# neggles/neurosis

Hardware: AMD Instinct MI355X
Metric: train images/sec (node) SDXL 1024^2 (higher is better)
Workload: dtype bf16

## Files before the change

include/neurosis_hip.h:

```cpp
#ifndef NEUROSIS_HIP_H
#define NEUROSIS_HIP_H

#ifdef __cplusplus
extern "C" {
#endif

const char* nk_last_error(void);
int nk_abi_version(void);

int nk_linear_fwd(const void* x, const void* w, const float* bias, const void* residual, void* y,
                  int M, int N, int K, long ldx, long ldw, long ldr, long ldy, float alpha, void* stream);
int nk_linear_dgrad(const void* dy, const void* w, const void* dx_add, void* dx, int M, int N, int K,
                    long lddy, long ldw, long ldadd, long lddx, void* stream);
long nk_linear_fwd_geglu_ok(int M, int I, int K);
int nk_linear_fwd_geglu(const void* x, const void* w, const float* bias, void* u, void* h, int M, int I, int K, long ldx, long ldw, long ldu,
                        long ldh, void* stream);
int nk_linear_dgrad_geglu(const void* dy, const void* w, const void* u, void* du, int M, int N, int I, long lddy, long ldw, long ldu,
                          long lddu, void* stream);
int nk_linear_fwd_geglu_s(const void* x, const void* w, const float* bias, void* s, void* h, int M, int I, int K, long ldx, long ldw, long lds,
                          long ldh, void* stream);
int nk_linear_dgrad_geglu_s(const void* dy, const void* w, const void* s, void* du, int M, int N, int I, long lddy, long ldw, long lds,
                            long lddu, void* stream);
int nk_linear_wgrad(const void* dy, const void* x, float* dw, int M, int N, int K, long lddy, long ldx,
                    long lddw, int accumulate, void* stream);
// ... 84 lines not shown
long nk_layernorm_ws_floats(int M, int C);
int nk_rmsnorm_fwd(const void* x, const float* gamma, void* y, int M, int C, float eps, void* stream);
int nk_layernorm_bwd(const void* dy, const void* x, const float* gamma, const float* mean, const float* rstd,
                     const void* dx_add, void* dx, float* dgamma, float* dbeta, float* ws, int M, int C, int accumulate, void* stream);
#define NK_COLPART_MAX 32
typedef struct NkColpartBatch {
  const float* part[NK_COLPART_MAX];
  float* dgamma[NK_COLPART_MAX];
  float* dbeta[NK_COLPART_MAX];
  int nrows[NK_COLPART_MAX];
  int C[NK_COLPART_MAX];
  int accumulate[NK_COLPART_MAX];
  int n;
} NkColpartBatch;
long nk_layernorm_part_rows(int M);
int nk_layernorm_bwd_rows(const void* dy, const void* x, const float* gamma, const float* mean, const float* rstd,
                          const void* dx_add, void* dx, float* part, int M, int C, void* stream);
int nk_colpart_reduce_batch(const NkColpartBatch* b, void* stream);
int nk_layernorm_bwd_dx(const void* dy, const void* x, const float* gamma, const float* mean, const float* rstd,
                        const void* dx_add, void* dx, int M, int C, void* stream);
int nk_layernorm_bwd_params(const void* dy, const void* x, const float* mean, const float* rstd, float* dgamma,
                            float* dbeta, float* ws, int M, int C, int accumulate, void* stream);

int nk_geglu_fwd(const void* u, void* y, long M, int I, void* stream);
int nk_geglu_bwd(const void* dy, const void* u, void* du, long M, int I, void* stream);
int nk_geglu_fwd_s(const void* u, void* y, void* s, long M, int I, void* stream);
int nk_geglu_bwd_s(const void* dy, const void* s, void* du, long M, int I, void* stream);

int nk_silu_fwd(const void* x, void* y, long n, void* stream);
int nk_silu_bwd(const void* dy, const void* x, void* dx, long n, void* stream);

int nk_dropout(const void* x, const void* residual, void* y, long rows, int cols, long ld_x, long ld_res, long ld_y, const void* token,
               int site, int thr, float scale, void* stream);
int nk_dropout_draw(void* state, void* token, void* stream);

int nk_add(const void* a, const void* b, void* out, long n, void* stream);

int nk_cat_channels(const void* a, const void* b, void* out, long rows, int Ca, int Cb, void* stream);
int nk_split_channels(const void* src, void* a, void* b, long rows, int Ca, int Cb, void* stream);

int nk_upsample2x_bwd(const void* dup, void* dx, int N, int H, int W, int C, void* stream);
int nk_upsample2x_fwd(const void* x, void* up, int N, int H, int W, int C, void* stream);
int nk_avgpool2x_fwd(const void* x, void* y, int N, int H, int W, int C, void* stream);
int nk_avgpool2x_bwd(const void* dy, void* dx, int N, int H, int W, int C, void* stream);

int nk_nchw_to_nhwc(const void* src, int src_is_f32, void* dst, int N, int C, int HW, int Cpad, float scale,
// ... 119 lines not shown
```

neurosis_amd/lib.py:

```python
from __future__ import annotations

import ctypes as C
import os
from pathlib import Path

import torch

CSRC = Path(__file__).resolve().parent / "csrc"
LIB_PATH = CSRC / "libneurosis_hip.so"

vp, i32, i64, f32 = C.c_void_p, C.c_int, C.c_long, C.c_float


class NkConvDesc(C.Structure):
    _fields_ = [(n, i32) for n in ("N", "H", "W", "Cin", "Cout", "KH", "KW", "stride", "pad_t", "pad_l", "Ho", "Wo", "upsample")]


class NkAttnDesc(C.Structure):
    _fields_ = (
        [(n, i32) for n in ("B", "H", "Lq", "Lk", "D")]
        + [(n, i64) for n in ("sq", "sk", "sv", "so", "bq", "bk", "bv", "bo", "sdq", "sdk", "sdv", "sdo", "bdq", "bdk", "bdv", "bdo")]
        + [("scale", f32), ("causal", i32)]
    )


NK_COLPART_MAX = 32


class NkColpartBatch(C.Structure):
    _fields_ = [("part", vp * NK_COLPART_MAX), ("dgamma", vp * NK_COLPART_MAX), ("dbeta", vp * NK_COLPART_MAX), ("nrows", i32 * NK_COLPART_MAX),
                ("C", i32 * NK_COLPART_MAX), ("accumulate", i32 * NK_COLPART_MAX), ("n", i32)]


cdp, adp = C.POINTER(NkConvDesc), C.POINTER(NkAttnDesc)

SIGNATURES: dict[str, list] = {
    "nk_linear_fwd": [vp, vp, vp, vp, vp, i32, i32, i32, i64, i64, i64, i64, f32, vp],
    "nk_linear_dgrad": [vp, vp, vp, vp, i32, i32, i32, i64, i64, i64, i64, vp],
    "nk_linear_dgrad_geglu": [vp, vp, vp, vp, i32, i32, i32, i64, i64, i64, i64, vp],
    "nk_linear_fwd_geglu": [vp, vp, vp, vp, vp, i32, i32, i32, i64, i64, i64, i64, vp],
    "nk_linear_fwd_geglu_s": [vp, vp, vp, vp, vp, i32, i32, i32, i64, i64, i64, i64, vp],
    "nk_linear_dgrad_geglu_s": [vp, vp, vp, vp, i32, i32, i32, i64, i64, i64, i64, vp],
    "nk_linear_wgrad": [vp, vp, vp, i32, i32, i32, i64, i64, i64, i32, vp],
    "nk_linear_fwd_batched": [C.POINTER(vp), C.POINTER(vp), C.POINTER(vp), i32, i32, i32, i32, i64, i64, i64, vp],
    "nk_linear_wgrad_batched": [C.POINTER(vp), C.POINTER(vp), C.POINTER(vp), C.POINTER(vp), i32, i32, i32, i32, i64, i64, i64, i32, vp],
    "nk_linear_wgrad_bias": [vp, vp, vp, vp, i32, i32, i32, i64, i64, i64, i32, vp],
    "nk_conv2d_wgrad_bias": [cdp, vp, vp, vp, vp, i32, vp],
    "nk_conv2d_fwd": [cdp, vp, vp, vp, vp, vp, vp, vp],
    "nk_conv2d_fwd_stats": [cdp, vp, vp, vp, vp, vp, vp, vp, i32, vp],
    "nk_conv_weight_flip": [vp, vp, i32, i32, i32, vp],
    "nk_conv3x3_few_channels_fwd": [vp, vp, vp, vp, i32, i32, i32, i32, i32, vp],
    "nk_conv2d_dgrad": [cdp, vp, vp, vp, vp],
    "nk_conv2d_dgrad_flipped": [cdp, vp, vp, vp, vp],
    "nk_conv2d_wgrad": [cdp, vp, vp, vp, i32, vp],
# ... 2 lines not shown
    "nk_attention_bwd_causal": [adp, vp, vp, vp, vp, vp, vp, vp, vp, vp, vp],
    "nk_attention_relbias_fwd": [adp, vp, vp, vp, vp, vp, vp],
    "nk_softmax_rows": [vp, i64, i32, vp],
    "nk_softmax_rows_bwd": [vp, vp, i64, i32, f32, vp],
    "nk_groupnorm_fwd": [vp, vp, vp, vp, vp, vp, vp, i32, i32, i32, i32, f32, i32, vp],
    "nk_groupnorm_sums": [vp, vp, vp, i32, i32, i32, i32, vp],
    "nk_groupnorm_sums_from_parts": [vp, vp, vp, i32, i32, i32, vp],
    "nk_groupnorm_apply": [vp, vp, vp, vp, vp, vp, vp, i32, i32, i32, i32, f32, i32, vp],
    "nk_groupnorm_bwd": [vp, vp, vp, vp, vp, vp, vp, vp, vp, vp, vp, i32, i32, i32, i32, i32, i32, vp],
    "nk_groupnorm_mod_fwd": [vp, vp, vp, vp, vp, vp, vp, vp, i32, i32, i32, i32, f32, i32, vp],
    "nk_groupnorm_mod_apply": [vp, vp, vp, vp, vp, vp, vp, vp, i32, i32, i32, i32, f32, i32, vp],
    "nk_groupnorm_mod_bwd": [vp, vp, vp, vp, vp, vp, vp, vp, vp, vp, vp, vp, vp, i32, i32, i32, i32, i32, i32, vp],
    "nk_layernorm_fwd": [vp, vp, vp, vp, vp, vp, i32, i32, f32, vp],
    "nk_rmsnorm_fwd": [vp, vp, vp, i32, i32, f32, vp],
    "nk_layernorm_bwd": [vp, vp, vp, vp, vp, vp, vp, vp, vp, vp, i32, i32, i32, vp],
    "nk_layernorm_bwd_dx": [vp, vp, vp, vp, vp, vp, vp, i32, i32, vp],
    "nk_layernorm_bwd_rows": [vp, vp, vp, vp, vp, vp, vp, vp, i32, i32, vp],
    "nk_colpart_reduce_batch": [C.POINTER(NkColpartBatch), vp],
    "nk_layernorm_bwd_params": [vp, vp, vp, vp, vp, vp, vp, i32, i32, i32, vp],
    "nk_geglu_fwd": [vp, vp, i64, i32, vp],
    "nk_geglu_bwd": [vp, vp, vp, i64, i32, vp],
    "nk_geglu_fwd_s": [vp, vp, vp, i64, i32, vp],
    "nk_geglu_bwd_s": [vp, vp, vp, i64, i32, vp],
    "nk_silu_fwd": [vp, vp, i64, vp],
    "nk_gelu_fwd": [vp, vp, i64, i32, vp],
    "nk_gated_gelu_tanh_fwd": [vp, vp, i64, i32, vp],
    "nk_gelu_bwd": [vp, vp, vp, i64, i32, vp],
    "nk_embedding_bwd": [vp, vp, i64, vp, vp, i32, i32, i32, i32, i32, i32, vp],
    "nk_gather_rows_bwd": [vp, i64, vp, vp, i32, i32, i32, vp],
    "nk_wgrad_few_rows": [vp, i64, vp, i64, vp, i64, i32, i32, i32, i32, vp],
    "nk_vq_search": [vp, i64, vp, vp, vp, i64, i32, i32, vp],
    "nk_vq_code_stats": [vp, vp, i64, vp, vp, i64, i32, i32, vp],
    "nk_vq_quantize": [vp, vp, vp, i64, vp, vp, vp, i64, i32, i32, i32, vp],
    "nk_leaky_relu_fwd": [vp, vp, i64, f32, vp],
    "nk_leaky_relu_bwd": [vp, vp, vp, i64, f32, vp],
    "nk_maxpool2x2_fwd": [vp, vp, i32, i32, i32, i32, vp],
    "nk_maxpool2x2_bwd": [vp, vp, vp, i32, i32, i32, i32, vp],
    "nk_maxpool_fwd": [vp, vp, i32, i32, i32, i32, i32, i32, vp],
    "nk_maxpool_bwd": [vp, vp, vp, i32, i32, i32, i32, i32, i32, vp],
    "nk_lpips_layer_fwd": [vp, vp, vp, vp, vp, i32, i32, i32, f32, i32, vp],
    "nk_lpips_layer_bwd": [vp, vp, vp, vp, vp, i32, i32, i32, f32, vp],
    "nk_batchnorm_fwd": [vp, vp, vp, vp, vp, vp, vp, vp, vp, i64, i32, f32, f32, f32, vp],
    "nk_batchnorm_bwd": [vp, vp, vp, vp, vp, vp, vp, vp, vp, vp, i64, i32, f32, i32, vp],
    "nk_batchnorm_eval": [vp, vp, vp, vp, vp, vp, vp, i64, i32, f32, f32, vp],
    "nk_silu_bwd": [vp, vp, vp, i64, vp],
    "nk_add": [vp, vp, vp, i64, vp],
# ... 20 lines not shown
    "nk_sample_denoise": [vp, vp, vp, vp, f32, vp, i32, i32, i32, i32, i32, vp],
    "nk_sample_euler_step": [vp, vp, vp, vp, vp, vp, f32, vp, vp, i32, i32, i32, i32, i32, vp],
    "nk_adamw_flat": [vp, vp, vp, vp, vp, i64, f32, f32, f32, f32, f32, i32, f32, vp],
    "nk_ema_flat": [vp, vp, i64, f32, vp],
    "nk_debug_raise_health": [vp],
    "nk_debug_stamp": [vp, vp],
    "nk_debug_launch_log": [i32],
    "nk_health_clear": [],
    "nk_health_export": [vp, vp],
    "nk_health_import": [vp, vp],
    "nk_adafactor_init": [vp, vp],
    "nk_adafactor_chunk": [vp, vp],
    "nk_came_chunk": [vp, vp],
    "nk_adamw8bit_step": [vp, vp],
}

SIZE_QUERIES: dict[str, list] = {
    "nk_groupnorm_ws_floats": [i32, i32, i32, i32],
    "nk_groupnorm_sums_ws_floats": [i32, i32, i32],
    "nk_conv2d_stats_tiles": [cdp, i32],
    "nk_conv2d_dgrad_flipped_ok": [cdp],
    "nk_linear_fwd_geglu_ok": [i32, i32, i32],
    "nk_layernorm_ws_floats": [i32, i32],
    "nk_layernorm_part_rows": [i32],
    "nk_colsum_ws_floats": [i64, i32],
    "nk_batchnorm_ws_floats": [i64, i32],
    "nk_lpips_layer_ws_floats": [i32, i32],
    "nk_attention_bwd_ws_floats": [adp],
    "nk_vq_search_ws_floats": [i64, i32],
    "nk_vq_quantize_ws_floats": [i64],
    "nk_adafactor_tensor_bytes": [],
    "nk_came_tensor_bytes": [],
    "nk_adamw8bit_tensor_bytes": [],
    "nk_gemm_sk_status": [],
    "nk_health_status": [],
    "nk_debug_launch_names": [C.c_char_p, i64],
}

_lib = None


class NkError(RuntimeError):
    pass


def load() -> C.CDLL:
# ... 48 lines not shown
```

neurosis_amd/models/diffusion.py:

```python
from __future__ import annotations

import os
from contextlib import contextmanager, nullcontext
from math import ceil
from typing import Callable, Optional

import torch
from torch import Tensor, nn

from .. import ops
from ..modules.diffusion import Denoiser, DiffusionLoss, OpenAIWrapper, UNetModel
from ..nn import FlatParamStore
from .autoencoder import AutoencoderKL


class PrecomputedConditioner(nn.Module):

    def forward(self, batch: dict, force_zero_embeddings=None) -> dict:
        zeroed = set(force_zero_embeddings or ())
        out = {}
        for k in ("crossattn", "vector", "concat"):
            if k in batch and batch[k] is not None:
                out[k] = torch.zeros_like(batch[k]) if k in zeroed else batch[k]
        return out
# ... 106 lines not shown
        if self.optimizer is not None and self._torch_optimizer is None:
            self.configure_optimizers()
        self.stream_optimizer = self.stream_optimizer
        return self.store

    @property
    def stream_optimizer(self) -> bool:
        return self._stream_optimizer

    @stream_optimizer.setter
    def stream_optimizer(self, on: bool) -> None:
        if on and self.trainable_embedders():
            raise NotImplementedError("stream_optimizer (the update streamed block by block behind backward) does not drive the text towers' groups")
        if on and getattr(self, "_torch_optimizer", None) is not None:
            from ..optimizers import CAME, AdamW8bit

            if isinstance(self._torch_optimizer, (CAME, AdamW8bit)):
                raise NotImplementedError(f"DiffusionEngine: stream_optimizer (the update streamed block by block behind backward) needs the fused "
                                          f"Adafactor, not {type(self._torch_optimizer).__name__}")
        self._stream_optimizer = bool(on)
        unet = getattr(getattr(self, "model", None), "diffusion_model", None)
        if unet is None or getattr(self, "store", None) is None:
            return
        if on:
            if unet.grad_ready_hook is None:
                unet.grad_ready_hook = self._grads_ready
        elif unet.grad_ready_hook == self._grads_ready:
            unet.grad_ready_hook = None

    def _block_boundaries(self) -> list:
        unet = self.model.diffusion_model
        index = {id(p): i for i, p in enumerate(self.store.params)}
        tops = [unet.time_embed, getattr(unet, "label_emb", None), *unet.input_blocks, unet.middle_block, *unet.output_blocks, unet.out]
        out = []
        for m in tops:
            if m is None:
                continue
            idx = [index[id(p)] for p in m.parameters() if id(p) in index]
            if idx:
                out.append(min(idx))
        return sorted(set(out))

    def _grads_ready(self, module: nn.Module) -> None:
        af = getattr(self, "adafactor", None)
        if af is None or not self.stream_optimizer or not self._last_micro_batch or not self.store.master.is_cuda:
            return
# ... 271 lines not shown
```

neurosis_amd/modules/diffusion/openaimodel.py:

```python
from __future__ import annotations

import os

from typing import Callable, List, Optional, Union

import torch
from torch import Tensor, nn

from ... import ops
from ...nn import Conv2d, FlatParamStore, apply_module, as_tokens, linear_module_fwd
from ...ops import BF16, Img
from ..attention import SpatialTransformer, zero_module


def conv_nd(dims: int, *args, **kwargs) -> nn.Module:
    if dims != 2:
        raise ValueError(f"unsupported dimensions: {dims} (the MI355X path implements 2-D convolutions)")
    return Conv2d(*args, **kwargs)


class TimestepBlock(nn.Module):

    def forward(self, x: Tensor, emb: Tensor):
        raise NotImplementedError("TimestepBlock is an interface: subclasses implement forward(x, emb)")
# ... 7 lines not shown
        for layer in self:
            if isinstance(layer, TimestepBlock):
                x, b = layer.fwd(x, emb)
                bwds.append(("emb", b))
            elif isinstance(layer, SpatialTransformer):
                x, b = layer.fwd(x, context, need_dctx=dctx_sink is not None)
                bwds.append(("ctx", b))
            elif isinstance(layer, (Conv2d, Upsample, Downsample)):
                x, b = layer.fwd(x, need_dx=not (first and getattr(self, "_nk_input_block", False)))
                bwds.append(("plain", b))
            elif isinstance(layer, nn.Identity):
                continue
            else:
                raise NotImplementedError(f"TimestepEmbedSequential: unsupported layer {type(layer).__name__}")
            first = False

        def bwd(dy: Tensor):
            demb = None
            for kind, b in reversed(bwds):
                if dy is None:
                    break
                if kind == "emb":
                    dy, de = b(dy)
                    demb = de if demb is None else ops.add(demb, de)
                elif kind == "ctx":
                    dy, dc = b(dy)
                    if dctx_sink is not None and dc is not None:
                        dctx_sink(dc)
                else:
                    dyi, _ = b(dy)
                    dy = None if dyi is None else dyi.t
            bwds.clear()
            return dy, demb

        return x, bwd

    def forward(self, x: Tensor, emb: Tensor, context: Optional[Tensor] = None, image_only_indicator=None, time_context=None, num_video_frames=None):
        ins = [x, emb] if context is None else [x, emb, context]
        ops.dropout_open(self)

        def run(x, emb, context=None):
            img = Img.from_nchw(x)
            out, bwd = self.fwd(img, as_tokens(emb), None if context is None else as_tokens(context))

            def bwd2(g):
                dx, demb = bwd(Img.from_nchw(g).t)
                res = (Img(dx, img.N, img.H, img.W).to_nchw(), None if demb is None else demb.view(emb.shape))
# ... 117 lines not shown
        if isinstance(skip, nn.Identity):
            s, b_skip = x.t, None
        elif skip.kernel_size == 1:
            s, b_skip = ops.linear_fwd(x.t, skip.weight, skip.bias)
        else:
            si, b_skip3 = skip.fwd(x, upsample=self._up)
            s, b_skip = si.t, (lambda g: b_skip3(g)[0].t)
        b_up = None
        if self._up and (b_skip is None or skip.kernel_size == 1):
            sup, b_up = ops.upsample2x_fwd(Img(s, x.N, x.H, x.W))
            s = sup.t
        if b_skip is None and b_res is None and b_up is None:
            return s, None

        def bwd(dy: Tensor) -> Tensor:
            if b_up is not None:
                dy = b_up(dy)
            if b_skip is not None:
                dy = b_skip(dy)
            return dy if b_res is None else b_res(dy)

        return s, bwd

    def _fwd(self, x: Img, emb: Tensor):
        gn1, gn2 = self.in_layers[0], self.out_layers[0]
        ssn = self.use_scale_shift_norm
        h1, b_gn1 = ops.groupnorm_fwd(x, gn1.weight, gn1.bias, 32, gn1.eps, silu=True)
        b_pool = None
        if self._down:
            h1, b_pool = ops.avgpool2x_fwd(h1)
        es, b_es = ops.silu_fwd(emb)
        eo, b_eo = linear_module_fwd(self.emb_layers[1], es)
        h2, b_c1 = self.in_layers[2].fwd(h1, rowvec=None if ssn else eo, upsample=self._up, stats_groups=32)
        if ssn:
            h3, b_gn2 = ops.groupnorm_mod_fwd(h2, gn2.weight, gn2.bias, eo, 32, gn2.eps, silu=True)
        else:
            h3, b_gn2 = ops.groupnorm_fwd(h2, gn2.weight, gn2.bias, 32, gn2.eps, silu=True)
        b_drop = None
        if self.training and self.dropout_p > 0.0:
            _, b_drop = ops.dropout_fwd(h3.t, self.dropout_p, ops.dropout_site(self), inplace=True)
        s, b_skip = self._skip_fwd(x)
        out, b_c2 = self.out_layers[3].fwd(h3, residual=s, stats_groups=32)

        def bwd(dy: Tensor):
            dh3, _ = b_c2(dy)
            dh2 = b_gn2(dh3.t if b_drop is None else b_drop(dh3.t, inplace=True))
            if ssn:
                dh2, deo = dh2
                dh1, _ = b_c1(dh2)
            else:
                dh1, deo = b_c1(dh2)
            dh1 = dh1.t if b_pool is None else b_pool(dh1.t)
            dxs = dy if b_skip is None else b_skip(dy)
            dx = b_gn1(dh1, dxs)
            demb = b_es(b_eo(deo))
            return dx, demb

        return out, bwd

    def fwd(self, x: Img, emb: Tensor):
        if not (self.use_checkpoint and ops.recording()):
            return self._fwd(x, emb)
        out, _ = self._fwd(x, emb)
        tok = ops.dropout_token(required=False)

        def bwd(dy: Tensor):
            with ops.dropout_token_scope(tok):
                _, b = self._fwd(x, emb)
            return b(dy)

        return out, bwd

    def forward(self, x: Tensor, emb: Tensor) -> Tensor:
        ops.dropout_open(self)

        def run(x, emb):
            img = Img.from_nchw(x)
            out, bwd = self.fwd(img, as_tokens(emb))

            def bwd2(g):
                dx, demb = bwd(Img.from_nchw(g).t)
                return Img(dx, img.N, img.H, img.W).to_nchw(), demb.view(emb.shape)

            return out.to_nchw(), bwd2

        return apply_module(run, [x, emb], self)


class Timestep(nn.Module):

    def __init__(self, dim: int):
        super().__init__()
        self.dim = dim

    def forward(self, t: Tensor) -> Tensor:
        return ops.timestep_embedding(t, self.dim)


class UNetModel(nn.Module):

    def __init__(
        self,
        in_channels: int,
        model_channels: int,
        out_channels: int,
        num_res_blocks: int,
        attention_resolutions,
        dropout: float = 0.0,
        channel_mult=(1, 2, 4, 8),
# ... 101 lines not shown
            res(ch, ch),
        )

        self.output_blocks = nn.ModuleList([])
        for level, mult in list(enumerate(channel_mult))[::-1]:
            for i in range(self.num_res_blocks[level] + 1):
                ich = input_block_chans.pop()
                layers = [res(ch + ich, model_channels * mult)]
                ch = model_channels * mult
                if ds in attention_resolutions:
                    disabled_sa = disable_self_attentions[level] if disable_self_attentions is not None else False
                    if num_attention_blocks is None or i < num_attention_blocks[level]:
                        layers.append(make_st(ch, transformer_depth[level], disabled_sa))
                if level and i == self.num_res_blocks[level]:
                    out_ch = ch
                    layers.append(res(ch, out_ch, up=True) if resblock_updown else Upsample(ch, conv_resample, dims=dims, out_channels=out_ch))
                    ds //= 2
                self.output_blocks.append(TimestepEmbedSequential(*layers))

        self.out = nn.Sequential(nn.GroupNorm(32, ch), nn.SiLU(), zero_module(conv_nd(dims, model_channels, out_channels, 3, padding=1)))
        self.input_blocks[0]._nk_input_block = True
        self.grad_ready_hook: Optional[Callable[[nn.Module], None]] = None
        self._nk_graphs = None

    def _mlp_fwd(self, seq: nn.Sequential, x: Tensor, need_dx: bool):
        a, b0 = linear_module_fwd(seq[0], x, need_dx=need_dx)
        s, b1 = ops.silu_fwd(a)
        o, b2 = linear_module_fwd(seq[2], s)
        return o, (lambda g: b0(b1(b2(g))))

    def set_recompute(self, policy: Optional[str]) -> "UNetModel":
        from ..attention import BasicTransformerBlock

        if policy not in (None, "norms"):
            raise ValueError(f"recompute policy must be None or 'norms', got {policy!r}")
        for m in self.modules():
            if isinstance(m, BasicTransformerBlock):
                m.recompute = policy
        self._nk_graphs = None
        return self

    def _project_context(self, context: Tensor) -> None:
        from ..attention import BasicTransformerBlock
        from ...nn import adjacent

        if getattr(self, "_nk_cross", None) is None:
            self._nk_cross = [blk.attn2 for blk in self.modules() if isinstance(blk, BasicTransformerBlock)]
        groups = {}
        for att in self._nk_cross:
            wk, wv = att.to_k.weight, att.to_v.weight
            if wk.shape[1] != context.shape[1] or not adjacent(wk, wv):
                continue
            groups.setdefault((wk.shape[0], wk.shape[1]), []).append(att)
        for (inner, cdim), atts in groups.items():
            if len(atts) < 2:
                continue
            ws = [torch.as_strided(ops.shadow(a.to_k.weight), (2 * inner, cdim), (cdim, 1)) for a in atts]
            outs = ops.gemm_nt_batched([context] * len(atts), ws)
            for a, kv in zip(atts, outs):
                a._nk_kv = (kv, context)

    def fwd_graphed(self, x: Img, timesteps: Tensor, context: Optional[Tensor], y: Optional[Tensor], need_dctx: bool = False, need_dy: bool = False):
        from ...graphs import ChainGraphs, frozen_stamp, graphs_enabled

        if not x.t.is_cuda or not graphs_enabled():
            return self.fwd(x, timesteps, context, y, need_dctx, need_dy)
        if self._nk_graphs is None:
            self._nk_graphs = ChainGraphs(self.out[2].weight, hook=lambda: self.grad_ready_hook)
        N, H, W = x.N, x.H, x.W
        return self._nk_graphs.run(lambda t, ts, c, yy: self.fwd(Img(t, N, H, W), ts, c, yy, need_dctx, need_dy), [x.t, timesteps, context, y],
                                   extra_key=(N, H, W, frozen_stamp(self), self.training, need_dctx, need_dy))

    def fwd(self, x: Img, timesteps: Tensor, context: Optional[Tensor], y: Optional[Tensor], need_dctx: bool = False, need_dy: bool = False):
        hook_raw = self.grad_ready_hook
        need_dctx = bool(need_dctx) and context is not None
        need_dy = bool(need_dy) and y is not None and self.num_classes is not None
        if self.training and self.dropout > 0.0:
            ops.dropout_open(self)
        t_emb = ops.timestep_embedding(timesteps, self.model_channels)
        emb, b_time = self._mlp_fwd(self.time_embed, t_emb, need_dx=False)
        b_label = None
        if self.num_classes is not None:
            lab, b_label = self._mlp_fwd(self.label_emb[0], y, need_dx=need_dy)
            emb = ops.add(emb, lab)
        if context is not None:
            self._project_context(context)
        dctx = [None]

        def sink(dc: Tensor) -> None:
            dctx[0] = dc if dctx[0] is None else ops.add(dctx[0], dc)

        sink_ = sink if need_dctx else None
        hs: List[Img] = []
        tape = []
        h = x
        for module in self.input_blocks:
            h, b = module.fwd(h, emb, context, sink_)
            hs.append(h)
            tape.append((module, b))
        h, b_mid = self.middle_block.fwd(h, emb, context, sink_)
        out_tape = []
        for module in self.output_blocks:
            h, b_cat = ops.cat_fwd(h, hs.pop())
            h, b = module.fwd(h, emb, context, sink_)
            out_tape.append((module, b, b_cat))
        gn = self.out[0]
        hn, b_gn = ops.groupnorm_fwd(h, gn.weight, gn.bias, 32, gn.eps, silu=True)
        out, b_conv = self.out[2].fwd(hn)

# ... 17 lines not shown
                if de is not None:
                    demb = de if demb is None else ops.add(demb, de)

            skips = []
            for module, b, b_cat in reversed(out_tape):
                dh, de = b(dh)
                acc_emb(de)
                dh, dskip = b_cat(dh)
                skips.append(dskip)
                if hook:
                    hook(module)
            out_tape.clear()
            dh, de = b_mid(dh)
            acc_emb(de)
            if hook:
                hook(self.middle_block)
            for module, b in reversed(tape):
                dh = ops.add(dh, skips.pop())
                dh, de = b(dh)
                acc_emb(de)
                if hook:
                    hook(module)
            tape.clear()
            dy = None
            if b_label is not None:
                dy = b_label(demb)
                if hook:
                    hook(self.label_emb)
            b_time(demb)
            if hook:
                hook(self.time_embed)
            ops.join_wgrad_stream(self.out[2].weight)
            if need_dctx or need_dy:
                return dh, dctx[0], dy
            return dh

        return out, bwd

    def forward(self, x: Tensor, timesteps: Optional[Tensor] = None, context: Optional[Tensor] = None, y: Optional[Tensor] = None, **kwargs) -> Tensor:
        if (y is not None) != (self.num_classes is not None):
            raise ValueError(f"UNetModel.forward: this network has no label embedding (num_classes=None) but was given y of shape {tuple(y.shape)}")
        if y is not None:
            assert y.shape[0] == x.shape[0]
        N, Cin, H, W = x.shape
        ins = [x, timesteps, context, y]

# ... 24 lines not shown
```

neurosis_amd/ops.py:

```python
from __future__ import annotations

import ctypes as C
import os
import threading
import weakref
from dataclasses import dataclass
from typing import Callable, Optional

import torch
from torch import Tensor

from . import lib
from .lib import NkAttnDesc, NkConvDesc, call, query

BF16 = torch.bfloat16


class EngineState:

    _live = weakref.WeakSet()

    def __init__(self, wgrad_stream=None):
        self.grad_accumulate = False
        self.assume_zeroed = False
# ... 728 lines not shown
         Cc, wgrad_mode(table), _stream())


def gather_rows_bwd(dsel: Tensor, idx: Tensor, L: int) -> Tensor:
    _check2d(dsel, "dsel")
    B, Cc = dsel.shape
    if idx.shape != (B,) or idx.dtype != torch.int64 or not idx.is_contiguous():
        raise ValueError("gather_rows_bwd: idx must be a dense int64 [B] tensor")
    dx = torch.empty(B * L, Cc, dtype=BF16, device=dsel.device)
    call("nk_gather_rows_bwd", dsel.data_ptr(), dsel.stride(0), idx.data_ptr(), dx.data_ptr(), B, L, Cc, _stream())
    return dx


def wgrad_few_rows(x: Tensor, dy: Tensor, dw: Tensor, accumulate: bool) -> None:
    _check2d(x, "x")
    _check2d(dy, "dy")
    M, K = x.shape
    N = dy.shape[1]
    if dy.shape[0] != M or dw.shape != (K, N) or dw.dtype != torch.float32 or dw.stride(1) != 1:
        raise ValueError(f"wgrad_few_rows: bad shapes {tuple(x.shape)} {tuple(dy.shape)} {tuple(dw.shape)}")
    call("nk_wgrad_few_rows", x.data_ptr(), x.stride(0), dy.data_ptr(), dy.stride(0), dw.data_ptr(), dw.stride(0), M, K, N, int(accumulate), _stream())


def leaky_relu_fwd(x: Tensor, slope: float = 0.2):
    y = torch.empty_like(x)
    call("nk_leaky_relu_fwd", x.data_ptr(), y.data_ptr(), x.numel(), float(slope), _stream())

    def bwd(dy: Tensor) -> Tensor:
        dx = torch.empty_like(dy)
        call("nk_leaky_relu_bwd", dy.data_ptr(), y.data_ptr(), dx.data_ptr(), dy.numel(), float(slope), _stream())
        return dx

    return y, bwd


def maxpool2x2_fwd(x: Img):
    y = torch.empty(x.N * (x.H // 2) * (x.W // 2), x.C, dtype=BF16, device=x.t.device)
    call("nk_maxpool2x2_fwd", x.t.data_ptr(), y.data_ptr(), x.N, x.H, x.W, x.C, _stream())

    def bwd(dy: Tensor) -> Tensor:
        dx = torch.empty_like(x.t)
        call("nk_maxpool2x2_bwd", dy.data_ptr(), x.t.data_ptr(), dx.data_ptr(), x.N, x.H, x.W, x.C, _stream())
        return dx

    return Img(y, x.N, x.H // 2, x.W // 2), bwd

# ... 72 lines not shown
         _p(running_var), _ws(nws, x.device).data_ptr(), M, Cc, float(eps), float(momentum), float(slope), _stream())

    def bwd(dy: Tensor) -> Tensor:
        dx = torch.empty_like(x)
        call("nk_batchnorm_bwd", dy.data_ptr(), x.data_ptr(), y.data_ptr(), weight.data_ptr(), mean.data_ptr(), rstd.data_ptr(), dx.data_ptr(),
             grad_flat(weight).data_ptr(), grad_flat(bias).data_ptr(), _ws(nws, x.device).data_ptr(), M, Cc, float(slope), int(state_of(weight).grad_accumulate),
             _stream())
        return dx

    return y, bwd


def batchnorm_eval(x: Tensor, weight: Tensor, bias: Tensor, running_mean: Tensor, running_var: Tensor, eps: float = 1e-5, slope: float = 1.0) -> Tensor:
    _check2d(x, "x")
    if not x.is_contiguous():
        raise ValueError("batchnorm: x must be dense")
    M, Cc = x.shape
    y = torch.empty_like(x)
    call("nk_batchnorm_eval", x.data_ptr(), weight.data_ptr(), bias.data_ptr(), running_mean.data_ptr(), running_var.data_ptr(), y.data_ptr(),
         _ws(Cc + 64, x.device).data_ptr(), M, Cc, float(eps), float(slope), _stream())
    return y


def silu_fwd(x: Tensor):
    y = torch.empty_like(x)
    call("nk_silu_fwd", x.data_ptr(), y.data_ptr(), x.numel(), _stream())

    def bwd(dy: Tensor):
        dx = torch.empty_like(x)
        call("nk_silu_bwd", dy.data_ptr(), x.data_ptr(), dx.data_ptr(), x.numel(), _stream())
        return dx

    return y, bwd


_dropout = threading.local()
_dropout_states: dict = {}


def _as_i64(v: int) -> int:
    v &= (1 << 64) - 1
    return v - (1 << 64) if v >= (1 << 63) else v


def _dropout_state_tensor(device=None) -> Tensor:
    dev = torch.device("cuda", torch.cuda.current_device()) if device is None else torch.device(device)
    if dev.type != "cuda":
        raise ValueError(f"dropout: the counter lives on a GPU, got device {dev}")
    idx = torch.cuda.current_device() if dev.index is None else dev.index
    st = _dropout_states.get(idx)
    if st is None:
        if capturing():
            raise RuntimeError("dropout: the first draw on a device cannot happen inside a hipGraph capture (it allocates the counter)")
        st = _dropout_states[idx] = torch.tensor([_as_i64(torch.initial_seed()), 0], dtype=torch.int64, device=torch.device("cuda", idx))
    return st

# ... 353 lines not shown
```

Baseline: 27.50.

## Batch ResBlock timestep-embedding projections into one grouped few-row linear kernel

Adds a grouped few-row linear kernel that computes the SiLU of the timestep embedding once and projects it through every ResBlock's emb linear in a single launch. In the backward pass it can defer the per-block embedding dgrads and reduce them with one slab-partitioned kernel plus a sum kernel, replacing many small GEMM, SiLU and add launches. It is on by default (NK_ROWS_BATCH=1), and the deferred dgrad path runs when the mode is 2. The cost is extra plumbing through per-module state and graph cache keys, plus a workspace allocation for the partial sums.

```diff
diff --git a/include/neurosis_hip.h b/include/neurosis_hip.h
--- a/include/neurosis_hip.h
+++ b/include/neurosis_hip.h
@@ -130,6 +130,22 @@
 int nk_layernorm_bwd_params(const void* dy, const void* x, const float* mean, const float* rstd, float* dgamma,
                             float* dbeta, float* ws, int M, int C, int accumulate, void* stream);
 
+#define NK_ROWS_MAX_R 8
+#define NK_ROWS_MAX_PROBLEMS 32
+typedef struct NkRowsTable {
+  const void* w[NK_ROWS_MAX_PROBLEMS];
+  const float* bias[NK_ROWS_MAX_PROBLEMS];
+  void* y[NK_ROWS_MAX_PROBLEMS];
+  long ldw[NK_ROWS_MAX_PROBLEMS];
+  long ldy[NK_ROWS_MAX_PROBLEMS];
+  int N[NK_ROWS_MAX_PROBLEMS];
+  int n;
+} NkRowsTable;
+long nk_rows_linear_ok(int R, int K, int count);
+long nk_rows_linear_dgrad_ws_floats(long total_rows, int R, int K);
+int nk_rows_linear_fwd(const NkRowsTable* t, const void* x, long ldx, void* xact, long ldxa, int R, int K, int act, void* stream);
+int nk_rows_linear_dgrad_sum(const NkRowsTable* t, const void* x, long ldx, void* dx, long lddx, float* ws, int R, int K, int act, void* stream);
+
 int nk_geglu_fwd(const void* u, void* y, long M, int I, void* stream);
 int nk_geglu_bwd(const void* dy, const void* u, void* du, long M, int I, void* stream);
 int nk_geglu_fwd_s(const void* u, void* y, void* s, long M, int I, void* stream);
diff --git a/neurosis_amd/csrc/rows_linear.hip b/neurosis_amd/csrc/rows_linear.hip
--- /dev/null
+++ b/neurosis_amd/csrc/rows_linear.hip
@@ -0,0 +1,239 @@
+#include "../../include/neurosis_hip.h"
+#include "nk_common.h"
+#include <stdio.h>
+
+#define RL_THREADS 256
+#define RL_FWD_ROWS 16
+#define RL_SLAB 64
+#define RL_SUM_WAVES 16
+#define RL_PLAN_TEXT 160
+
+__device__ __forceinline__ void rl_locate(const NkRowsTable& t, int g, int& p, int& row) {
+  p = 0;
+  while (p < t.n && g >= t.N[p]) g -= t.N[p++];
+  row = g;
+}
+
+template <int R>
+__global__ __launch_bounds__(RL_THREADS) void rows_linear_fwd_kernel(const NkRowsTable t, const bf16_t* __restrict__ x, long ldx,
+                                                                       bf16_t* __restrict__ xact, long ldxa, int K, int act, int total) {
+  extern __shared__ uint4_t sx[];
+  const int K8 = K >> 3;
+  for (int i = threadIdx.x; i < R * K8; i += RL_THREADS) {
+    const int r = i / K8, c = i - r * K8;
+    uint4_t v = *(const uint4_t*)(x + r * ldx + c * 8);
+    if (act) {
+      float f[8];
+      unpack8(v, f);
+#pragma unroll
+      for (int e = 0; e < 8; ++e) f[e] = silu_f(f[e]);
+      v = pack8(f);
+      if (blockIdx.x == 0 && xact) *(uint4_t*)(xact + r * ldxa + c * 8) = v;
+    }
+    sx[i] = v;
+  }
+  __syncthreads();
+  const int lane = threadIdx.x & 63;
+  const int wave = __builtin_amdgcn_readfirstlane(threadIdx.x >> 6);
+  const int g0 = blockIdx.x * RL_FWD_ROWS;
+  const int g1 = min(g0 + RL_FWD_ROWS, total);
+  for (int g = g0 + wave; g < g1; g += RL_THREADS / 64) {
+    int p, n;
+    rl_locate(t, g, p, n);
+    const bf16_t* wr = (const bf16_t*)t.w[p] + (long)n * t.ldw[p];
+    float acc[R];
+#pragma unroll
+    for (int r = 0; r < R; ++r) acc[r] = 0.f;
+    for (int c = lane; c < K8; c += 64) {
+      float wf[8];
+      unpack8(*(const uint4_t*)(wr + c * 8), wf);
+#pragma unroll
+      for (int r = 0; r < R; ++r) {
+        float xf[8];
+        unpack8(sx[r * K8 + c], xf);
+#pragma unroll
+        for (int e = 0; e < 8; ++e) acc[r] = fmaf(xf[e], wf[e], acc[r]);
+      }
+    }
+    float mine = 0.f;
+#pragma unroll
+    for (int r = 0; r < R; ++r) {
+      const float s = wave_sum(acc[r]);
+      if (lane == r) mine = s;
+    }
+    if (lane < R) {
+      if (t.bias[p]) mine += t.bias[p][n];
+      ((bf16_t*)t.y[p])[(long)lane * t.ldy[p] + n] = f2bf(mine);
+    }
+  }
+}
+
+template <int R>
+__global__ __launch_bounds__(RL_THREADS) void rows_linear_dgrad_part_kernel(const NkRowsTable t, float* __restrict__ part, int K, int total) {
+  __shared__ float sdy[RL_SLAB][R];
+  const int g0 = blockIdx.x * RL_SLAB;
+  const int rows = min(RL_SLAB, total - g0);
+  for (int j = threadIdx.x; j < rows; j += RL_THREADS) {
+    int p, n;
+    rl_locate(t, g0 + j, p, n);
+    const bf16_t* dy = (const bf16_t*)t.y[p];
+#pragma unroll
+    for (int r = 0; r < R; ++r) sdy[j][r] = bf2f(dy[(long)r * t.ldy[p] + n]);
+  }
+  __syncthreads();
+  const int c = blockIdx.y * RL_THREADS + threadIdx.x;
+  if (c >= (K >> 3)) return;
+  float acc[R][8];
+#pragma unroll
+  for (int r = 0; r < R; ++r)
+#pragma unroll
+    for (int e = 0; e < 8; ++e) acc[r][e] = 0.f;
+  int p, n;
+  rl_locate(t, g0, p, n);
+  const bf16_t* wr = (const bf16_t*)t.w[p] + (long)n * t.ldw[p] + c * 8;
+#pragma unroll 4
+  for (int j = 0; j < rows; ++j) {
+    float wf[8];
+    unpack8(*(const uint4_t*)wr, wf);
+#pragma unroll
+    for (int r = 0; r < R; ++r) {
+      const float d = sdy[j][r];
+#pragma unroll
+      for (int e = 0; e < 8; ++e) acc[r][e] = fmaf(d, wf[e], acc[r][e]);
+    }
+    wr += t.ldw[p];
+    if (++n == t.N[p] && j + 1 < rows) {
+      ++p;
+      n = 0;
+      wr = (const bf16_t*)t.w[p] + c * 8;
+    }
+  }
+  float* out = part + ((long)blockIdx.x * R) * K + c * 8;
+#pragma unroll
+  for (int r = 0; r < R; ++r) {
+    *(float4_t*)(out + (long)r * K) = float4_t{acc[r][0], acc[r][1], acc[r][2], acc[r][3]};
+    *(float4_t*)(out + (long)r * K + 4) = float4_t{acc[r][4], acc[r][5], acc[r][6], acc[r][7]};
+  }
+}
+
+__global__ __launch_bounds__(64 * RL_SUM_WAVES) void rows_linear_dgrad_sum_kernel(const float* __restrict__ part, int nslab, int R, int K,
+                                                                                    const bf16_t* __restrict__ x, long ldx, int act,
+                                                                                    bf16_t* __restrict__ dx, long lddx) {
+  __shared__ float4_t red[RL_SUM_WAVES][64];
+  const int lane = threadIdx.x & 63, wave = threadIdx.x >> 6;
+  const int k = (blockIdx.x * 64 + lane) * 4, r = blockIdx.y;
+  const bool live = k < K;
+  float4_t s = {0.f, 0.f, 0.f, 0.f};
+  if (live) {
+    const int per = (nslab + RL_SUM_WAVES - 1) / RL_SUM_WAVES;
+    const int s0 = wave * per, s1 = min(s0 + per, nslab);
+    for (int i = s0; i < s1; ++i) s += *(const float4_t*)(part + ((long)i * R + r) * K + k);
+  }
+  red[wave][lane] = s;
+  __syncthreads();
+  if (wave != 0 || !live) return;
+  for (int w = 1; w < RL_SUM_WAVES; ++w) s += red[w][lane];
+  float f[4] = {s.x, s.y, s.z, s.w};
+  if (act) {
+    float xf[4];
+    unpack4(*(const uint2_t*)(x + r * ldx + k), xf);
+#pragma unroll
+    for (int e = 0; e < 4; ++e) f[e] *= dsilu_f(xf[e]);
+  }
+  uint2_t o;
+  o.x = pack2bf(f[0], f[1]);
+  o.y = pack2bf(f[2], f[3]);
+  *(uint2_t*)(dx + r * lddx + k) = o;
+}
+
+static bool rl_aligned16(const void* p) { return p && ((uintptr_t)p & 15) == 0; }
+
+extern "C" long nk_rows_linear_ok(int R, int K, int count) {
+  return R >= 1 && R <= NK_ROWS_MAX_R && K >= 8 && (K & 7) == 0 && (long)R * K * 2 <= 65536 && count >= 1 && count <= NK_ROWS_MAX_PROBLEMS;
+}
+
+static long rl_check_table(const NkRowsTable* t, int R, int K) {
+  if (!t || !nk_rows_linear_ok(R, K, t->n)) {
+    nk_set_error(__FILE__, __LINE__, "rows_linear: 1 <= R <= 8, K % 8 == 0, R * K <= 32768 and 1 <= n <= NK_ROWS_MAX_PROBLEMS expected");
+    return -1;
+  }
+  long total = 0;
+  for (int i = 0; i < t->n; ++i) {
+    if (!rl_aligned16(t->w[i]) || t->N[i] < 1 || t->ldw[i] < K || (t->ldw[i] & 7) || !t->y[i] || ((uintptr_t)t->y[i] & 1) || t->ldy[i] < t->N[i]) {
+      nk_set_error(__FILE__, __LINE__, "rows_linear: a table entry needs a 16-byte aligned weight, ldw >= K and a multiple of 8, N >= 1, an output and ldy >= N");
+      return -1;
+    }
+    total += t->N[i];
+  }
+  if (total > 0x7fffffffL / 8) {
+    nk_set_error(__FILE__, __LINE__, "rows_linear: too many weight rows");
+    return -1;
+  }
+  return total;
+}
+
+extern "C" long nk_rows_linear_dgrad_ws_floats(long total_rows, int R, int K) {
+  if (total_rows < 1 || R < 1 || K < 1) return -1;
+  return (total_rows + RL_SLAB - 1) / RL_SLAB * R * K;
+}
+
+template <int R>
+static void rl_launch_fwd(const NkRowsTable* t, const void* x, long ldx, void* xact, long ldxa, int K, int act, int total, hipStream_t s) {
+  hipLaunchKernelGGL(rows_linear_fwd_kernel<R>, dim3((total + RL_FWD_ROWS - 1) / RL_FWD_ROWS), dim3(RL_THREADS), (size_t)R * K * 2, s, *t,
+                     (const bf16_t*)x, ldx, (bf16_t*)xact, ldxa, K, act, total);
+}
+template <int R>
+static void rl_launch_part(const NkRowsTable* t, float* ws, int K, int total, hipStream_t s) {
+  hipLaunchKernelGGL(rows_linear_dgrad_part_kernel<R>, dim3((total + RL_SLAB - 1) / RL_SLAB, ((K >> 3) + RL_THREADS - 1) / RL_THREADS),
+                     dim3(RL_THREADS), 0, s, *t, ws, K, total);
+}
+
+#define RL_FOR_R(R, CALL)                                                  \
+  switch (R) {                                                             \
+    case 1: CALL(1); break; case 2: CALL(2); break; case 3: CALL(3); break; \
+    case 4: CALL(4); break; case 5: CALL(5); break; case 6: CALL(6); break; \
+    case 7: CALL(7); break; default: CALL(8); break;                       \
+  }
+
+extern "C" int nk_rows_linear_fwd(const NkRowsTable* t, const void* x, long ldx, void* xact, long ldxa, int R, int K, int act, void* stream) {
+  const long total = rl_check_table(t, R, K);
+  if (total < 0) return NK_ERR_ARG;
+  NK_CHECK_ARG(act == 0 || act == 1);
+  NK_CHECK_ARG(rl_aligned16(x) && ldx >= K && (ldx & 7) == 0);
+  NK_CHECK_ARG(xact == nullptr || (act == 1 && rl_aligned16(xact) && ldxa >= K && (ldxa & 7) == 0));
+  if (nk_launch_log_mode() == 3) {
+    char line[RL_PLAN_TEXT];
+    snprintf(line, sizeof(line), "rows_linear_fwd grid=%ld,1,1 %d %d n=%d rows=%ld", (total + RL_FWD_ROWS - 1) / RL_FWD_ROWS, RL_THREADS, R * K * 2, t->n, total);
+    nk_launch_log_add("rows_linear_fwd", line);
+    return NK_OK;
+  }
+#define RL_CALL(RR) rl_launch_fwd<RR>(t, x, ldx, xact, ldxa, K, act, (int)total, (hipStream_t)stream)
+  RL_FOR_R(R, RL_CALL)
+#undef RL_CALL
+  return nk_check_launch("rows_linear_fwd");
+}
+
+extern "C" int nk_rows_linear_dgrad_sum(const NkRowsTable* t, const void* x, long ldx, void* dx, long lddx, float* ws, int R, int K, int act,
+                                        void* stream) {
+  const long total = rl_check_table(t, R, K);
+  if (total < 0) return NK_ERR_ARG;
+  NK_CHECK_ARG(act == 0 || act == 1);
+  NK_CHECK_ARG(dx && ((uintptr_t)dx & 7) == 0 && lddx >= K && (lddx & 3) == 0 && rl_aligned16(ws));
+  NK_CHECK_ARG(act == 0 || (x && ((uintptr_t)x & 7) == 0 && ldx >= K && (ldx & 3) == 0));
+  const int nslab = (int)((total + RL_SLAB - 1) / RL_SLAB);
+  if (nk_launch_log_mode() == 3) {
+    char line[RL_PLAN_TEXT];
+    snprintf(line, sizeof(line), "rows_linear_dgrad_part grid=%d,%d,1 %d n=%d rows=%ld", nslab, ((K >> 3) + RL_THREADS - 1) / RL_THREADS, RL_THREADS, t->n, total);
+    nk_launch_log_add("rows_linear_dgrad_part", line);
+    snprintf(line, sizeof(line), "rows_linear_dgrad_sum grid=%d,%d,1 %d slabs=%d", (K / 4 + 63) / 64, R, 64 * RL_SUM_WAVES, nslab);
+    nk_launch_log_add("rows_linear_dgrad_sum", line);
+    return NK_OK;
+  }
+#define RL_CALL(RR) rl_launch_part<RR>(t, ws, K, (int)total, (hipStream_t)stream)
+  RL_FOR_R(R, RL_CALL)
+#undef RL_CALL
+  if (int e = nk_check_launch("rows_linear_dgrad_part")) return e;
+  hipLaunchKernelGGL(rows_linear_dgrad_sum_kernel, dim3((K / 4 + 63) / 64, R), dim3(64 * RL_SUM_WAVES), 0, (hipStream_t)stream, (const float*)ws, nslab, R,
+                     K, (const bf16_t*)x, ldx, act, (bf16_t*)dx, lddx);
+  return nk_check_launch("rows_linear_dgrad_sum");
+}
diff --git a/neurosis_amd/lib.py b/neurosis_amd/lib.py
--- a/neurosis_amd/lib.py
+++ b/neurosis_amd/lib.py
@@ -30,6 +30,14 @@
 class NkColpartBatch(C.Structure):
     _fields_ = [("part", vp * NK_COLPART_MAX), ("dgamma", vp * NK_COLPART_MAX), ("dbeta", vp * NK_COLPART_MAX), ("nrows", i32 * NK_COLPART_MAX),
                 ("C", i32 * NK_COLPART_MAX), ("accumulate", i32 * NK_COLPART_MAX), ("n", i32)]
+
+
+NK_ROWS_MAX_R, NK_ROWS_MAX_PROBLEMS = 8, 32
+
+
+class NkRowsTable(C.Structure):
+    _fields_ = [("w", vp * NK_ROWS_MAX_PROBLEMS), ("bias", vp * NK_ROWS_MAX_PROBLEMS), ("y", vp * NK_ROWS_MAX_PROBLEMS), ("ldw", i64 * NK_ROWS_MAX_PROBLEMS),
+                ("ldy", i64 * NK_ROWS_MAX_PROBLEMS), ("N", i32 * NK_ROWS_MAX_PROBLEMS), ("n", i32)]
 
 
 cdp, adp = C.POINTER(NkConvDesc), C.POINTER(NkAttnDesc)
@@ -78,6 +86,8 @@
     "nk_geglu_bwd": [vp, vp, vp, i64, i32, vp],
     "nk_geglu_fwd_s": [vp, vp, vp, i64, i32, vp],
     "nk_geglu_bwd_s": [vp, vp, vp, i64, i32, vp],
+    "nk_rows_linear_fwd": [C.POINTER(NkRowsTable), vp, i64, vp, i64, i32, i32, i32, vp],
+    "nk_rows_linear_dgrad_sum": [C.POINTER(NkRowsTable), vp, i64, vp, i64, vp, i32, i32, i32, vp],
     "nk_silu_fwd": [vp, vp, i64, vp],
     "nk_gelu_fwd": [vp, vp, i64, i32, vp],
     "nk_gated_gelu_tanh_fwd": [vp, vp, i64, i32, vp],
@@ -144,6 +154,8 @@
     "nk_conv2d_dgrad_flipped_ok": [cdp],
     "nk_linear_fwd_geglu_ok": [i32, i32, i32],
     "nk_layernorm_ws_floats": [i32, i32],
+    "nk_rows_linear_ok": [i32, i32, i32],
+    "nk_rows_linear_dgrad_ws_floats": [i64, i32, i32],
     "nk_layernorm_part_rows": [i32],
     "nk_colsum_ws_floats": [i64, i32],
     "nk_batchnorm_ws_floats": [i64, i32],
diff --git a/neurosis_amd/models/diffusion.py b/neurosis_amd/models/diffusion.py
--- a/neurosis_amd/models/diffusion.py
+++ b/neurosis_amd/models/diffusion.py
@@ -152,6 +152,7 @@
         unet = getattr(getattr(self, "model", None), "diffusion_model", None)
         if unet is None or getattr(self, "store", None) is None:
             return
+        unet.defer_emb_dgrad = not on
         if on:
             if unet.grad_ready_hook is None:
                 unet.grad_ready_hook = self._grads_ready
diff --git a/neurosis_amd/modules/diffusion/openaimodel.py b/neurosis_amd/modules/diffusion/openaimodel.py
--- a/neurosis_amd/modules/diffusion/openaimodel.py
+++ b/neurosis_amd/modules/diffusion/openaimodel.py
@@ -53,7 +53,8 @@
                     break
                 if kind == "emb":
                     dy, de = b(dy)
-                    demb = de if demb is None else ops.add(demb, de)
+                    if de is not None:
+                        demb = de if demb is None else ops.add(demb, de)
                 elif kind == "ctx":
                     dy, dc = b(dy)
                     if dctx_sink is not None and dc is not None:
@@ -217,15 +218,20 @@
 
         return s, bwd
 
-    def _fwd(self, x: Img, emb: Tensor):
+    def _fwd(self, x: Img, emb: Tensor, pre=None):
         gn1, gn2 = self.in_layers[0], self.out_layers[0]
         ssn = self.use_scale_shift_norm
         h1, b_gn1 = ops.groupnorm_fwd(x, gn1.weight, gn1.bias, 32, gn1.eps, silu=True)
         b_pool = None
         if self._down:
             h1, b_pool = ops.avgpool2x_fwd(h1)
-        es, b_es = ops.silu_fwd(emb)
-        eo, b_eo = linear_module_fwd(self.emb_layers[1], es)
+        if pre is not None:
+            eo, es, deo_sink = pre
+            lin = self.emb_layers[1]
+            b_es, b_eo = ops.silu_bwd_of(emb), ops._linear_bwd(es, lin.weight, lin.bias, need_dx=deo_sink is None)
+        else:
+            es, b_es = ops.silu_fwd(emb)
+            eo, b_eo = linear_module_fwd(self.emb_layers[1], es)
         h2, b_c1 = self.in_layers[2].fwd(h1, rowvec=None if ssn else eo, upsample=self._up, stats_groups=32)
         if ssn:
             h3, b_gn2 = ops.groupnorm_mod_fwd(h2, gn2.weight, gn2.bias, eo, 32, gn2.eps, silu=True)
@@ -248,14 +254,21 @@
             dh1 = dh1.t if b_pool is None else b_pool(dh1.t)
             dxs = dy if b_skip is None else b_skip(dy)
             dx = b_gn1(dh1, dxs)
+            if pre is not None and deo_sink is not None:
+                b_eo(deo)
+                deo_sink(self, deo)
+                return dx, None
             demb = b_es(b_eo(deo))
             return dx, demb
 
         return out, bwd
 
     def fwd(self, x: Img, emb: Tensor):
+        pre = self.__dict__.pop("_nk_eo", None)
+        if pre is not None and pre[0] is not emb:
+            pre = None
         if not (self.use_checkpoint and ops.recording()):
-            return self._fwd(x, emb)
+            return self._fwd(x, emb, None if pre is None else pre[1:])
         out, _ = self._fwd(x, emb)
         tok = ops.dropout_token(required=False)
 
@@ -280,6 +293,22 @@
             return out.to_nchw(), bwd2
 
         return apply_module(run, [x, emb], self)
+
+
+class _EmbGrads:
+
+    def __init__(self, emb: Tensor):
+        self.emb = emb
+        self.items = []
+
+    def add(self, block: "ResBlock", deo: Tensor) -> None:
+        self.items.append((block.emb_layers[1].weight, deo))
+
+    def finish(self) -> Optional[Tensor]:
+        items, self.items = self.items, []
+        if not items:
+            return None
+        return ops.rows_linear_dgrad_sum([d for _, d in items], [ops.w2d(w) for w, _ in items], self.emb, act="silu")
 
 
 class Timestep(nn.Module):
@@ -427,6 +456,7 @@
         self.input_blocks[0]._nk_input_block = True
         self.grad_ready_hook: Optional[Callable[[nn.Module], None]] = None
         self._nk_graphs = None
+        self.defer_emb_dgrad = True
 
     def _mlp_fwd(self, seq: nn.Sequential, x: Tensor, need_dx: bool):
         a, b0 = linear_module_fwd(seq[0], x, need_dx=need_dx)
@@ -465,6 +495,22 @@
             for a, kv in zip(atts, outs):
                 a._nk_kv = (kv, context)
 
+    def _project_emb(self, emb: Tensor):
+        mode = ops.rows_batch_mode()
+        if not mode or not emb.is_cuda:
+            return None
+        if getattr(self, "_nk_res", None) is None:
+            self._nk_res = [m for m in self.modules() if isinstance(m, ResBlock)]
+        blocks = [m for m in self._nk_res if m.emb_layers[1].weight.shape[1] == emb.shape[1] and not (m.use_checkpoint and ops.recording())]
+        if len(blocks) < 2 or not ops.rows_linear_ok(emb, len(blocks)):
+            return None
+        lins = [m.emb_layers[1] for m in blocks]
+        eos, es = ops.rows_linear_fwd(emb, [ops.w2d(l.weight) for l in lins], [l.bias for l in lins], act="silu")
+        col = _EmbGrads(emb) if mode == 2 and self.defer_emb_dgrad else None
+        for m, eo in zip(blocks, eos):
+            m._nk_eo = (emb, eo, es, None if col is None else col.add)
+        return col
+
     def fwd_graphed(self, x: Img, timesteps: Tensor, context: Optional[Tensor], y: Optional[Tensor], need_dctx: bool = False, need_dy: bool = False):
         from ...graphs import ChainGraphs, frozen_stamp, graphs_enabled
 
@@ -474,7 +520,7 @@
             self._nk_graphs = ChainGraphs(self.out[2].weight, hook=lambda: self.grad_ready_hook)
         N, H, W = x.N, x.H, x.W
         return self._nk_graphs.run(lambda t, ts, c, yy: self.fwd(Img(t, N, H, W), ts, c, yy, need_dctx, need_dy), [x.t, timesteps, context, y],
-                                   extra_key=(N, H, W, frozen_stamp(self), self.training, need_dctx, need_dy))
+                                   extra_key=(N, H, W, frozen_stamp(self), self.training, need_dctx, need_dy, ops.rows_batch_mode(), self.defer_emb_dgrad))
 
     def fwd(self, x: Img, timesteps: Tensor, context: Optional[Tensor], y: Optional[Tensor], need_dctx: bool = False, need_dy: bool = False):
         hook_raw = self.grad_ready_hook
@@ -490,6 +536,7 @@
             emb = ops.add(emb, lab)
         if context is not None:
             self._project_context(context)
+        emb_grads = self._project_emb(emb)
         dctx = [None]
 
         def sink(dc: Tensor) -> None:
@@ -553,6 +600,8 @@
                 if hook:
                     hook(module)
             tape.clear()
+            if emb_grads is not None:
+                acc_emb(emb_grads.finish())
             dy = None
             if b_label is not None:
                 dy = b_label(demb)
diff --git a/neurosis_amd/ops.py b/neurosis_amd/ops.py
--- a/neurosis_amd/ops.py
+++ b/neurosis_amd/ops.py
@@ -774,6 +774,70 @@
     call("nk_wgrad_few_rows", x.data_ptr(), x.stride(0), dy.data_ptr(), dy.stride(0), dw.data_ptr(), dw.stride(0), M, K, N, int(accumulate), _stream())
 
 
+def rows_batch_mode() -> int:
+    v = os.environ.get("NK_ROWS_BATCH", "1")
+    return int(v) if v in ("0", "1", "2") else 1
+
+
+def rows_linear_ok(x: Tensor, n_problems: int) -> bool:
+    return x.dim() == 2 and x.dtype == BF16 and x.stride(1) == 1 and bool(query("nk_rows_linear_ok", x.shape[0], x.shape[1], n_problems))
+
+
+def rows_table(ws, biases, ys) -> lib.NkRowsTable:
+    n = len(ws)
+    if not (1 <= n <= lib.NK_ROWS_MAX_PROBLEMS) or len(biases) != n or len(ys) != n:
+        raise ValueError(f"rows_table: 1..{lib.NK_ROWS_MAX_PROBLEMS} problems with one bias (or None) and one output each, got {n}, {len(biases)}, {len(ys)}")
+    R, K = ys[0].shape[0], ws[0].shape[1]
+    t = lib.NkRowsTable()
+    for i, (w, b, y) in enumerate(zip(ws, biases, ys)):
+        _check2d(w, "w")
+        _check2d(y, "y")
+        N = w.shape[0]
+        if w.shape[1] != K or y.shape != (R, N):
+            raise ValueError(f"rows_table: problem {i}: weight {tuple(w.shape)} and rows {tuple(y.shape)} do not fit R = {R}, K = {K}")
+        if b is not None and (b.shape != (N,) or b.dtype != torch.float32 or not b.is_contiguous()):
+            raise ValueError(f"rows_table: problem {i}: the bias must be a dense fp32 [{N}] tensor")
+        t.w[i], t.bias[i], t.y[i] = w.data_ptr(), _p(b), y.data_ptr()
+        t.ldw[i], t.ldy[i], t.N[i] = w.stride(0), y.stride(0), N
+    t.n = n
+    return t
+
+
+def rows_linear_fwd(x: Tensor, ws, biases, act: str = "none", ys=None):
+    _check2d(x, "x")
+    R, K = x.shape
+    if act not in ("none", "silu"):
+        raise ValueError(f"rows_linear_fwd: act must be 'none' or 'silu', got {act!r}")
+    if ys is None:
+        ys = [torch.empty(R, w.shape[0], dtype=BF16, device=x.device) for w in ws]
+    if any(w.shape[1] != K for w in ws):
+        raise ValueError(f"rows_linear_fwd: every weight must be [N_i, {K}]")
+    xact = torch.empty(R, K, dtype=BF16, device=x.device) if act == "silu" else x
+    call("nk_rows_linear_fwd", C.byref(rows_table(ws, biases, ys)), x.data_ptr(), x.stride(0), xact.data_ptr() if act == "silu" else None, xact.stride(0),
+         R, K, int(act == "silu"), _stream())
+    return ys, xact
+
+
+def rows_linear_dgrad_sum(dys, ws, x: Optional[Tensor] = None, act: str = "none") -> Tensor:
+    if act not in ("none", "silu") or (act == "silu" and x is None):
+        raise ValueError("rows_linear_dgrad_sum: act is 'none', or 'silu' with the forward's input x")
+    t = rows_table(ws, [None] * len(ws), dys)
+    R, K = dys[0].shape[0], ws[0].shape[1]
+    if x is not None:
+        _check2d(x, "x")
+        if x.shape != (R, K):
+            raise ValueError(f"rows_linear_dgrad_sum: x must be [{R}, {K}], got {tuple(x.shape)}")
+    dx = torch.empty(R, K, dtype=BF16, device=dys[0].device)
+    total = sum(w.shape[0] for w in ws)
+    ws_floats = query("nk_rows_linear_dgrad_ws_floats", total, R, K)
+    if ws_floats < 0:
+        raise ValueError(f"rows_linear_dgrad_sum: bad sizes (rows {total}, R {R}, K {K})")
+    part = _ws(ws_floats, dx.device)
+    call("nk_rows_linear_dgrad_sum", C.byref(t), _p(x) if act == "silu" else None, x.stride(0) if x is not None else 0, dx.data_ptr(), dx.stride(0),
+         part.data_ptr(), R, K, int(act == "silu"), _stream())
+    return dx
+
+
 def leaky_relu_fwd(x: Tensor, slope: float = 0.2):
     y = torch.empty_like(x)
     call("nk_leaky_relu_fwd", x.data_ptr(), y.data_ptr(), x.numel(), float(slope), _stream())
@@ -892,16 +956,19 @@
     return y
 
 
-def silu_fwd(x: Tensor):
-    y = torch.empty_like(x)
-    call("nk_silu_fwd", x.data_ptr(), y.data_ptr(), x.numel(), _stream())
-
+def silu_bwd_of(x: Tensor):
     def bwd(dy: Tensor):
         dx = torch.empty_like(x)
         call("nk_silu_bwd", dy.data_ptr(), x.data_ptr(), dx.data_ptr(), x.numel(), _stream())
         return dx
 
-    return y, bwd
+    return bwd
+
+
+def silu_fwd(x: Tensor):
+    y = torch.empty_like(x)
+    call("nk_silu_fwd", x.data_ptr(), y.data_ptr(), x.numel(), _stream())
+    return y, silu_bwd_of(x)
 
 
 _dropout = threading.local()
```

Result: no change. 27.50, median of 2 (+0.0%).
